# songrise/HyperNeRF-torch

Measured on AMD Instinct MI355X. Metric: ray-samples/sec (fwd+bwd+Adam), whole job; per-GPU = value/n_gpus, higher is better.
Workload: dtype bf16

## Files before the change

hypernerf-torch_amd/csrc/hn_mlp.hip:

```cpp
#include "hn_common.h"
#include <algorithm>
#include <type_traits>

#ifdef HN_PROF
#define HN_STAMP(code)                                                                          \
  do {                                                                                          \
    if (prof_on && prof_n < 2040) {                                                             \
      unsigned long long t__;                                                                   \
      __builtin_amdgcn_sched_barrier(0);                                                        \
      asm volatile("s_memtime %0\n\ts_waitcnt lgkmcnt(0)" : "=s"(t__)::"memory");               \
      __builtin_amdgcn_sched_barrier(0);                                                        \
      if (lane == 0) { prof_buf[2 * prof_n] = (code); prof_buf[2 * prof_n + 1] = (long long)t__; } \
      ++prof_n;                                                                                 \
    }                                                                                           \
  } while (0)
#else
#define HN_STAMP(code) do {} while (0)
#endif

template <int WAVES>
struct WStream {
  const char* g;
  char* lds;
  int ctr;
  int nchunks;
  int wave, lane;

  HN_DEV void issue(int c) {
    const char* src = g + (size_t)c * (HN_CHUNK_UNITS * 1024);
    char* dst = lds + (c & 1) * (HN_CHUNK_UNITS * 1024);
    if constexpr (WAVES == 8) {
      if (wave >= 4) {
        int u0 = wave - 4;
        asm volatile("" : "+s"(u0));
#pragma unroll
        for (int i = 0; i < HN_CHUNK_UNITS / 4; ++i) {
          const int unit = u0 + i * 4;
          __builtin_amdgcn_global_load_lds(
              (const __attribute__((address_space(1))) void*)(src + unit * 1024 + lane * 16),
              (__attribute__((address_space(3))) void*)(dst + unit * 1024), 16, 0, 0);
        }
      }
      return;
    }
#pragma unroll
    for (int i = 0; i < HN_CHUNK_UNITS / WAVES; ++i) {
      const int unit = wave + i * WAVES;
      __builtin_amdgcn_global_load_lds(
          (const __attribute__((address_space(1))) void*)(src + unit * 1024 + lane * 16),
          (__attribute__((address_space(3))) void*)(dst + unit * 1024), 16, 0, 0);
    }
  }
  HN_DEV void start() {
    ctr = 0;
    __syncthreads();
    issue(0);
  }
  HN_DEV const char* take(int n) {
    if ((ctr & (HN_CHUNK_UNITS - 1)) + n > HN_CHUNK_UNITS) ctr = (ctr + HN_CHUNK_UNITS - 1) & ~(HN_CHUNK_UNITS - 1);
    if ((ctr & (HN_CHUNK_UNITS - 1)) == 0) {
      const int c = ctr / HN_CHUNK_UNITS;
      asm volatile("s_waitcnt vmcnt(0)" ::: "memory");
      __syncthreads();
      if (c + 1 < nchunks) issue(c + 1);
    }
    const char* p = lds + (((ctr / HN_CHUNK_UNITS) & 1) * HN_CHUNK_UNITS + (ctr & (HN_CHUNK_UNITS - 1))) * 1024;
    ctr += n;
    return p;
  }
};

#define HN_INV2PI_HI 0.15915494309189535f
#define HN_INV2PI_LO ((float)(0.15915494309189535 - (double)0.15915494309189535f))
// ... 424 lines not shown
    }
    __builtin_amdgcn_sched_barrier(0);
#pragma unroll
    for (int u = 0; u < N; ++u) {
      if (t < NT) {
        acc[t & 1] = hn_mfma_bf16(q[u % D], cur[u], acc[t & 1]);
        if (u + D < N) q[u % D] = *reinterpret_cast<const bf16x8*>(wl + (u + D) * 1024);
      }
      if (t > 0) {
#pragma unroll
        for (int e = 0; e < PER_SLOT; ++e) {
          const int k = u * PER_SLOT + e;
          if (k < SHARES)
            hn_epilogue_share<TRAIN, NT, S8>(k, tp, acc[tp & 1], nxt + tp * 2, bits, out_base, mask_base, lane);
        }
      }
      __builtin_amdgcn_sched_barrier(0);
    }
  }
#pragma unroll
  for (int i = 0; i < NT * 2; ++i) cur[i] = nxt[i];
}

template <bool BF16, int AUXG, bool EXTRA, bool TRAIN, bool S8 = false>
__global__ __launch_bounds__(ModeT<BF16>::WAVES * 64, BF16 ? 2 : 1) void hn_mlp_fwd_kernel(const HnMlpArgs a) {
  using M = ModeT<BF16>;
  constexpr int SX = S8 ? 1 : 0;
  static_assert(!(S8 && (EXTRA || !TRAIN || !BF16)), "the 8-bit stash exists for the render-level bf16 training builds only");
  if constexpr (S8) asm volatile("s_setreg_imm32_b32 hwreg(HW_REG_MODE, 23, 1), 1");
  using Frag = typename M::Frag;
  extern __shared__ __attribute__((aligned(16))) char smem[];
  const int lane = threadIdx.x & 63;
  const int wave = __builtin_amdgcn_readfirstlane(threadIdx.x >> 6);
  const int r = lane & 31, h = lane >> 5;
  constexpr int PTS = M::WAVES * 32;
  const int ntiles = (a.n_points + PTS - 1) / PTS;
  hn_timeline_begin(a.timeline);
#ifdef HN_PROF
  long long* prof_buf = reinterpret_cast<long long*>(a.prof);
  const bool prof_on = prof_buf != nullptr && blockIdx.x == 0 && wave == 0;
  int prof_n = 0;
#endif

  WStream<M::WAVES> ws;
  ws.g = reinterpret_cast<const char*>(a.wstream);
  ws.lds = smem;
  ws.nchunks = a.n_chunks;
  ws.wave = wave;
// ... 17 lines not shown
    feat_lds[i] = e;
    if constexpr (BF16) dfeat_lds[i] = hn_derive_feat_fwd(e, a.n_comps, n_trig, with_lo);
  }
  __syncthreads();

  for (int tile = blockIdx.x; tile < ntiles; tile += gridDim.x) {
    const int blk = tile * M::WAVES + wave;
    const int p0 = blk * 32 + r;
    const bool valid = p0 < a.n_points;
    const int p = valid ? p0 : a.n_points - 1;
    const int ray = p / a.samples_per_ray;
    const bool wave_valid = blk * 32 < a.n_points;
    hn_stage_sources(srcv, a, p, ray, lane, rev, n_trig, with_lo);
    ws.start();

    HnOpWords w_next = hn_load_op(a.ops, 0, a.n_ops);
    for (int op = 0; op < a.n_ops; ++op) {
      const HnOpWords w = w_next;
      w_next = hn_load_op(a.ops, op + 1, a.n_ops);
      const int code = w[0];
      if (code == HN_OP_LAYER) {
        HN_STAMP(100 + op);
        const int K32 = w[1] & 255, nG = (w[1] >> 8) & 255, NT = (w[1] >> 16) & 255;
        const int act = (w[1] >> 24) & 15, flags = (w[1] >> 28) & 15;
        const float* bias = bias_lds + w[2];
        const bool do_mask = TRAIN && w[4] >= 0 && wave_valid && act != HN_ACT_SOFTPLUS;
        const bool do_stash = TRAIN && w[5] >= 0 && wave_valid;
        char* out_base = do_stash ? hn_slot_base<BF16, SX>(a, w[5], NT, blk) : nullptr;
        char* aux_base = (TRAIN && wave_valid) ? hn_slot_base<BF16, SX>(a, w[6], 2 * nG, blk) : nullptr;
        uint32_t* mask_base = do_mask ? hn_mask_base(a, w[4], (NT + 1) >> 1, blk, lane) : nullptr;
        const bool has_out = w_next[0] == HN_OP_OUT;
        const HnOpWords out_w = w_next;
        Frag aux[AUXG * 2 * M::STEPS32];
#pragma unroll
        for (int g = 0; g < AUXG; ++g) {
          if (g < nG) {
            if (EXTRA && (flags & HN_LAYER_DIRECT))
              hn_make_group<true>(aux + g * 2 * M::STEPS32, feat_lds + w[3] + 64 * g, dfeat_lds + w[3] + 64 * g, srcv,
                                  lane, a, p, ray);
            else
              hn_make_group<false>(aux + g * 2 * M::STEPS32, feat_lds + w[3] + 64 * g, dfeat_lds + w[3] + 64 * g, srcv,
                                   lane, a, p, ray);
            if (aux_base != nullptr) {
              hn_stash<BF16, SX>(aux + g * 2 * M::STEPS32, aux_base, 2 * g, lane);
              hn_stash<BF16, SX>(aux + (g * 2 + 1) * M::STEPS32, aux_base, 2 * g + 1, lane);
            }
          }
        }
        unsigned bits = 0;
// ... 3 lines not shown
                             wave_valid && do_stash == do_mask;
          if (plain && K32 == 4 && NT == 4) {
            if (do_stash) hn_layer_pipelined<4, 4, true, SX>(cur, nxt, bias, ws, out_base, mask_base, lane);
            else hn_layer_pipelined<4, 4, false, SX>(cur, nxt, bias, ws, out_base, mask_base, lane);
            continue;
          }
        }
#pragma unroll
        for (int t = 0; t < 8; ++t) {
          if (t < NT) {
            f32x16 acc;
            hn_init_acc(acc, bias, t, h);
            hn_gemm_k<BF16>(acc, cur, K32, ws);
#pragma unroll
            for (int g = 0; g < AUXG; ++g)
              if (g < nG) hn_gemm_blocks<BF16, 2>(acc, aux + g * 2 * M::STEPS32, ws);
            HN_STAMP(2);
            if (act == HN_ACT_RELU) {
#pragma unroll
              for (int i = 0; i < 16; ++i) {
                bits = hn_push_mask<BF16>(bits, acc[i]);
                acc[i] = __int_as_float(max(__float_as_int(acc[i]), 0));
              }
            } else if (act != HN_ACT_NONE) {
              hn_act_tile<BF16>(acc, act, __int_as_float(w[7]), __int_as_float(w[4]), bits);
            }
            if (has_out && t == 0 && h == 0 && valid) {
              const HnDst d = a.dst[out_w[1]];
              const int n = out_w[3];
#pragma unroll
              for (int i = 0; i < 4; ++i) {
                if (i < n) {
                  float y = acc[i];
                  if (out_w[4] == 1) y = 1.0f / (1.0f + expf(-y));
                  if (out_w[5] >= 0) {
                    const HnSrc sr = a.src[out_w[5]];
                    y = __fadd_rn(sr.ptr[(size_t)(sr.per_ray ? ray : p) * sr.ld + out_w[6] + i], y);
                  }
                  d.ptr[(size_t)p * d.ld + out_w[2] + i] = y;
                }
              }
            }
            if (has_out && t == 0 && h == 0 && out_w[7] > 0) {
              const int n = out_w[3];
#pragma unroll
              for (int i = 0; i < 4; ++i) {
                if (i < n) {
// ... 50 lines not shown
            if (t < NT) {
              if constexpr (BF16) {
#pragma unroll
                for (int s = 0; s < 2; ++s)
#pragma unroll
                  for (int j = 0; j < 8; ++j) {
                    const int row = 32 * t + 16 * s + hn_pi16(h, j);
                    if (row < n) d.ptr[(size_t)p * d.ld + w[2] + row] = (float)cur[2 * t + s][j];
                  }
              } else {
#pragma unroll
                for (int q = 0; q < 16; ++q) {
                  const int row = 32 * t + hn_rho(q, h);
                  if (row < n) d.ptr[(size_t)p * d.ld + w[2] + row] = cur[16 * t + q];
                }
              }
            }
        }
      }
    }
  }
  hn_timeline_end(a.timeline);
}

HN_DEV bool hn_prefetch_masks(const HnMlpArgs& a, const HnOpWords& wn, int blk, int lane, bool wave_valid,
                              unsigned* out) {
  if (wn[0] != HN_BOP_LAYER || wn[4] < 0) return false;
  const int NT = (wn[1] >> 16) & 255;
  const uint32_t* mb = hn_mask_base(a, wn[4], (NT + 1) >> 1, blk, lane);
#pragma unroll
  for (int dd = 0; dd < 4; ++dd)
    out[dd] = (2 * dd < NT) ? (wave_valid ? mb[dd * 64 + lane] : 0xffffffffu) : 0u;
  return true;
}

template <bool BF16, bool WIDE, bool S8 = false>
__global__ __launch_bounds__(ModeT<BF16>::WAVES * 64, BF16 ? 2 : 1) void hn_mlp_bwd_kernel(const HnMlpArgs a) {
  using M = ModeT<BF16>;
  constexpr int SZ = S8 ? 2 : 0;
  static_assert(!(S8 && WIDE) && !(S8 && !BF16), "the 8-bit stash exists for the render-level bf16 builds only");
  if constexpr (S8) asm volatile("s_setreg_imm32_b32 hwreg(HW_REG_MODE, 23, 1), 1");
  const float dz_scale = S8 ? ldexpf(1.0f, a.dz_scale_log2) : 1.0f;
  const float dz_unscale = S8 ? ldexpf(1.0f, -a.dz_scale_log2) : 1.0f;
  using Frag = typename M::Frag;
  extern __shared__ __attribute__((aligned(16))) char smem[];
  const int lane = threadIdx.x & 63;
  const int wave = __builtin_amdgcn_readfirstlane(threadIdx.x >> 6);
  const int r = lane & 31, h = lane >> 5;
  constexpr int PTS = M::WAVES * 32;
  const int ntiles = (a.n_points + PTS - 1) / PTS;
  HnFeat* feat_lds = reinterpret_cast<HnFeat*>(smem + 2 * HN_CHUNK_UNITS * 1024);
  HnDFeat* dfeat_lds = reinterpret_cast<HnDFeat*>(feat_lds + ((a.n_feat + 1) & ~1));
  float* srcv = reinterpret_cast<float*>(BF16 ? reinterpret_cast<char*>(dfeat_lds + a.n_feat)
                                              : reinterpret_cast<char*>(dfeat_lds)) + wave * (a.n_comps * 32);
  hn_timeline_begin(a.timeline);
#ifdef HN_PROF
  long long* prof_buf = reinterpret_cast<long long*>(a.prof);
  const bool prof_on = prof_buf != nullptr && blockIdx.x == 0 && wave == 0;
  int prof_n = 0;
#endif
// ... 63 lines not shown
            } else {
              d[i] = 0.0f;
            }
        } else {
#pragma unroll
          for (int i = 0; i < 4; ++i) d[i] = 0.0f;
        }
        Frag tmp[M::STEPS32];
        hn_zero_frags(tmp, M::STEPS32);
        if constexpr (BF16) {
#pragma unroll
          for (int i = 0; i < 4; ++i) tmp[0][i] = (__bf16)d[i];
        } else {
#pragma unroll
          for (int i = 0; i < 4; ++i) tmp[i] = d[i];
        }
        if (a.training && w[7] >= 0 && wave_valid) hn_stash<BF16, SZ>(tmp, hn_slot_base<BF16, SZ>(a, w[7], 1, blk), 0, lane);
#pragma unroll
        for (int s = 0; s < M::STEPS32; ++s) {
          if (to2) cur2[s] = tmp[s];
          else cur[s] = tmp[s];
        }
      } else if (WIDE && code == HN_BOP_LOAD_WIDE) {
        const int n = w[3] & 0xffff, NT = w[4], dact = (w[3] >> 16) & 15;
        const HnSrc s = a.src[w[1]];
        unsigned nbits = 0xffffffffu;
        char* dz_base = (a.training && wave_valid) ? hn_slot_base<BF16>(a, w[7], NT, blk) : nullptr;
        const bool has_mask = w[5] >= 0 && dact != HN_ACT_SOFTPLUS;
        const bool from_y = (dact == HN_ACT_ELU || dact == HN_ACT_SOFTPLUS) && wave_valid;
        const char* y_base = from_y ? hn_slot_base<BF16>(a, w[7], NT, blk) : nullptr;
#pragma unroll
        for (int t = 0; t < 8; ++t) {
          if (t < NT) {
            if (has_mask && !(t & 1)) {
              nbits = wave_valid ? ~hn_mask_base(a, w[5], (NT + 1) >> 1, blk, lane)[(t >> 1) * 64 + lane] : 0u;
            }
            f32x16 v;
            if (dact == 0) {
#pragma unroll
              for (int i = 0; i < 16; ++i) {
                const int row = 32 * t + hn_rho(i, h);
                const bool keep = hn_keep_mask(nbits, t & 1, i) != 0;
                v[i] = (valid && keep && row < n) ? s.ptr[(size_t)p * s.ld + w[2] + row] : 0.0f;
              }
            } else {
              const float p0 = __int_as_float(w[6]), p1 = __int_as_float(w[5]);
              f32x16 y = {0};
              if (y_base != nullptr) y = hn_unstash<BF16>(y_base, t, lane);
#pragma unroll
              for (int i = 0; i < 16; ++i) {
                const int row = 32 * t + hn_rho(i, h);
                const float g = (valid && row < n) ? s.ptr[(size_t)p * s.ld + w[2] + row] : 0.0f;
                float d = 1.0f;
                if (dact == HN_ACT_LEAKY_RELU) d = hn_keep_mask(nbits, t & 1, i) != 0 ? 1.0f : p0;
                else d = hn_dact_y<BF16>(dact, y[i], p0, p1);
                v[i] = g * d;
              }
            }
            hn_acc_to_frags(v, cur + t * M::STEPS32);
            if (dz_base != nullptr) hn_stash<BF16>(cur + t * M::STEPS32, dz_base, t, lane);
          }
        }
      } else if (code == HN_BOP_LAYER) {
        const int K32 = w[1] & 255, K32b = (w[1] >> 8) & 255, NT = (w[1] >> 16) & 255;
        const bool has_mask = w[4] >= 0;
        const bool do_stash = a.training && w[5] >= 0 && wave_valid;
        char* dz_base = do_stash ? hn_slot_base<BF16, SZ>(a, w[5], NT, blk) : nullptr;
        const int dact = w[2];
        const char* y_base = (!S8 && (dact == HN_ACT_ELU || dact == HN_ACT_SOFTPLUS) && wave_valid)
                                 ? hn_slot_base<BF16>(a, w[6], NT, blk) : nullptr;
        unsigned nbits = 0xffffffffu;
        unsigned mbits[4] = {0xffffffffu, 0xffffffffu, 0xffffffffu, 0xffffffffu};
        if (has_mask) {
          if (mnext_ready) {
#pragma unroll
            for (int dd = 0; dd < 4; ++dd) mbits[dd] = ~mnext[dd];
          } else {
            const uint32_t* mb = hn_mask_base(a, w[4], (NT + 1) >> 1, blk, lane);
#pragma unroll
            for (int dd = 0; dd < 4; ++dd)
              if (2 * dd < NT)
                mbits[dd] = wave_valid ? ~mb[dd * 64 + lane] : 0u;
          }
        }
        mnext_ready = false;
#pragma unroll
        for (int t = 0; t < 8; ++t) {
          if (t < NT) {
            f32x16 acc;
            hn_init_acc(acc, nullptr, t, h);
            hn_gemm_k<BF16>(acc, cur, K32, ws);
// ... 71 lines not shown
      for (int i = 0; i < 16; ++i) {
        const int slot = hn_rho(i, h);
        if (slot < a.n_dsrc) a.dsrc[(size_t)p0 * a.n_dsrc + slot] = S8 ? dacc[i] * dz_unscale : dacc[i];
      }
    }
    if (a.embed_reg_mask != 0 && wave_valid) {
      const long long erow = a.embed_idx[(blk * 32) / a.samples_per_ray];
#pragma unroll
      for (int i = 0; i < 16; ++i) {
        if (a.embed_reg_mask & (1 << i)) {
          float v = valid ? (S8 ? dacc[i] * dz_unscale : dacc[i]) : 0.0f;
#pragma unroll
          for (int m = 1; m < 32; m <<= 1) v += __shfl_xor(v, m, 64);
          const int col = a.embed_col[hn_rho(i, h)];
          if (r == 0 && col >= 0) {
            if (!S8 && a.embed_partial != nullptr) a.embed_partial[(size_t)blk * a.embed_dim + col] = v;
            else if (erow >= 0 && erow < a.embed_rows) atomicAdd(a.embed_grad + (size_t)erow * a.embed_dim + col, v);
          }
        }
      }
    }
  }
  hn_timeline_end(a.timeline);
}

#include "hn_pack.h"
template <bool BF16>
__global__ void hn_pack_kernel(const HnPackUnit* units, int n_units, const float* const* ptrs, char* out,
                               const HnPackBias* bias, int n_bias, float* bias_out) {
  hn_pack_one<BF16>(units, n_units, ptrs, out, bias, n_bias, bias_out, blockIdx.x * (blockDim.x >> 6) + (threadIdx.x >> 6));
}
template <bool BF16>
__global__ void hn_pack_multi_kernel(const HnPackTable tab) {
  hn_pack_block<BF16>(tab, (int)blockIdx.x);
}

template <class F>
HN_DEV void static_for4(F&& f) {
  f(std::integral_constant<int, 0>{});
  f(std::integral_constant<int, 1>{});
  f(std::integral_constant<int, 2>{});
  f(std::integral_constant<int, 3>{});
}
template <bool BF16>
struct DwFrag;
typedef __attribute__((ext_vector_type(4))) short s16x4;
// ... 505 lines not shown
  return 8;
}

#define HN_STR2(x) #x
#define HN_STR(x) HN_STR2(x)
extern "C" __attribute__((used)) const char hn_build_config_text[] =
    "HN_BUILD_CONFIG:" HN_STR(HN_WGRAD_STAGES) "," HN_STR(HN_WGRAD_MAXSLOT) ",0," HN_STR(HN_CHUNK_UNITS) ",1,1,"
    HN_STR(HN_BF16_WAVES) "," HN_STR(HN_WGRAD_AUX) ";";
extern "C" int hn_build_config(int32_t* out, int n) {
  const int32_t v[HN_BUILD_CONFIG_N] = {HN_WGRAD_STAGES, HN_WGRAD_MAXSLOT, 0, HN_CHUNK_UNITS,
                                        1,               1,                HN_BF16_WAVES, HN_WGRAD_AUX};
  for (int i = 0; i < n && i < HN_BUILD_CONFIG_N; ++i) out[i] = v[i];
  return HN_BUILD_CONFIG_N;
}

static void hn_allow_big_lds() {
  static bool done[64] = {};
  int dev = 0;
  if (hipGetDevice(&dev) != hipSuccess || dev < 0 || dev >= 64) dev = 0;
  if (done[dev]) return;
  done[dev] = true;
  const int big = 160 * 1024;
#define HN_BIG(k) (void)hipFuncSetAttribute((const void*)(k), hipFuncAttributeMaxDynamicSharedMemorySize, big)
  HN_BIG((hn_mlp_fwd_kernel<true, 2, false, true>)); HN_BIG((hn_mlp_fwd_kernel<true, 2, false, false>));
  HN_BIG((hn_mlp_fwd_kernel<true, 2, true, true>)); HN_BIG((hn_mlp_fwd_kernel<true, 2, true, false>));
  HN_BIG((hn_mlp_fwd_kernel<true, 3, false, true>)); HN_BIG((hn_mlp_fwd_kernel<true, 3, false, false>));
  HN_BIG((hn_mlp_fwd_kernel<true, 3, true, true>)); HN_BIG((hn_mlp_fwd_kernel<true, 3, true, false>));
  HN_BIG((hn_mlp_fwd_kernel<false, 3, true, true>)); HN_BIG((hn_mlp_fwd_kernel<false, 3, true, false>));
  HN_BIG((hn_mlp_fwd_kernel<true, 2, false, true, true>)); HN_BIG((hn_mlp_fwd_kernel<true, 3, false, true, true>));
  HN_BIG((hn_mlp_bwd_kernel<true, false, true>)); HN_BIG((hn_wgrad_kernel<true, true>));
#undef HN_BIG
  (void)hipFuncSetAttribute((const void*)hn_mlp_bwd_kernel<true, false>, hipFuncAttributeMaxDynamicSharedMemorySize, big);
  (void)hipFuncSetAttribute((const void*)hn_mlp_bwd_kernel<true, true>, hipFuncAttributeMaxDynamicSharedMemorySize, big);
  (void)hipFuncSetAttribute((const void*)hn_mlp_bwd_kernel<false, true>, hipFuncAttributeMaxDynamicSharedMemorySize, big);
  (void)hipFuncSetAttribute((const void*)hn_wgrad_kernel<true>, hipFuncAttributeMaxDynamicSharedMemorySize, big);
  (void)hipFuncSetAttribute((const void*)hn_wgrad_kernel<false>, hipFuncAttributeMaxDynamicSharedMemorySize, big);
}

extern "C" int hn_pack_units(int mode, const HnPackUnit* units, int n_units, const float* const* ptrs, void* wstream,
                             const HnPackBias* bias, int n_bias, float* bias_out, hnStream_t stream) {
  if (n_units < 0 || n_bias < 0) return -1;
  const int total = n_units + n_bias;
  if (total == 0) return 0;
  const int grid = (total + 3) / 4;
  if (mode == HN_MODE_BF16 || mode == HN_MODE_BF16_S8)
    hipLaunchKernelGGL(hn_pack_kernel<true>, dim3(grid), dim3(256), 0, (hipStream_t)stream, units, n_units, ptrs,
                       (char*)wstream, bias, n_bias, bias_out);
  else if (mode == HN_MODE_F32)
    hipLaunchKernelGGL(hn_pack_kernel<false>, dim3(grid), dim3(256), 0, (hipStream_t)stream, units, n_units, ptrs,
                       (char*)wstream, bias, n_bias, bias_out);
  else
    return -2;
  HN_CHECK_LAUNCH();
  return 0;
}

extern "C" int hn_pack_units_multi(int mode, const HnPackJob* jobs, int n_jobs, hnStream_t stream) {
  HnPackTable tab = {};
  int blocks = 0;
  const int rc = hn_pack_table_fill(jobs, n_jobs, tab, blocks);
  if (rc != 0) return rc;
  if (blocks == 0) return 0;
  if (mode == HN_MODE_BF16 || mode == HN_MODE_BF16_S8)
    hipLaunchKernelGGL(hn_pack_multi_kernel<true>, dim3(blocks), dim3(256), 0, (hipStream_t)stream, tab);
  else if (mode == HN_MODE_F32)
    hipLaunchKernelGGL(hn_pack_multi_kernel<false>, dim3(blocks), dim3(256), 0, (hipStream_t)stream, tab);
  else
    return -2;
  HN_CHECK_LAUNCH();
  return 0;
}

static int hn_check_args(const HnMlpArgs* a) {
  if (a == nullptr) return -1;
  if (a->n_points <= 0 || a->samples_per_ray <= 0 || a->n_ops <= 0 || a->n_chunks <= 0) return -2;
  if (a->ops == nullptr || a->wstream == nullptr) return -3;
  if (a->mode != HN_MODE_BF16 && a->mode != HN_MODE_F32 && a->mode != HN_MODE_BF16_S8) return -4;
  if (a->mode == HN_MODE_BF16_S8 && a->training && a->wide_ops != 0) return -4;
  if (a->mode == HN_MODE_BF16_S8 && (a->dz_scale_log2 < -60 || a->dz_scale_log2 > 60)) return -5;
  if (a->n_dsrc < 0 || a->n_dsrc > HN_DSRC_COMPS) return -5;
  if (a->n_bias < 0 || a->n_feat < 0 || a->n_comps < 0 || a->n_comps > HN_MAX_COMPS) return -5;
  if (a->max_groups < 0 || a->max_groups > 3) return -5;
  if (a->n_comps > 0 && a->comps == nullptr) return -3;
  return 0;
}

extern "C" int hn_mlp_workspace_bytes(const int32_t* ops_host, int n_ops, int backward, int mode, int64_t n_points,
                                      int64_t* stash_bytes, int64_t* mask_bytes) {
  if (ops_host == nullptr || stash_bytes == nullptr || mask_bytes == nullptr) return -1;
  if (n_ops <= 0 || n_points <= 0) return -2;
  if (mode != HN_MODE_BF16 && mode != HN_MODE_F32 && mode != HN_MODE_BF16_S8) return -4;
  const int64_t nblk = (n_points + 31) / 32;
  const int64_t tile = (mode == HN_MODE_BF16_S8 ? 1 : mode == HN_MODE_BF16 ? ModeT<true>::TILE_UNITS : ModeT<false>::TILE_UNITS) * 1024;
  int64_t sb = 0, mb = 0;
  auto stash = [&](int off_kib, int nt) {
    if (off_kib >= 0) sb = std::max<int64_t>(sb, (int64_t)(unsigned)off_kib * 1024 + nblk * nt * tile);
  };
  auto mask = [&](int off256, int nt_tiles) {
    if (off256 >= 0) mb = std::max<int64_t>(mb, (int64_t)(unsigned)off256 * 256 + nblk * ((nt_tiles + 1) >> 1) * 256);
  };
  for (int i = 0; i < n_ops; ++i) {
    const int32_t* w = ops_host + (size_t)i * HN_OP_WORDS;
    if (!backward) {
      if (w[0] == HN_OP_LAYER) {
        const int nG = (w[1] >> 8) & 255, NT = (w[1] >> 16) & 255, act = (w[1] >> 24) & 15;
        if (act != HN_ACT_SOFTPLUS) mask(w[4], NT);
        stash(w[5], NT);
        stash(w[6], 2 * nG);
      } else if (w[0] != HN_OP_OUT && w[0] != HN_OP_OUT_WIDE) {
        return -7;
      }
    } else {
      if (w[0] == HN_BOP_LOAD) {
        stash(w[7], 1);
      } else if (w[0] == HN_BOP_LOAD_WIDE) {
        if (((w[3] >> 16) & 15) != HN_ACT_SOFTPLUS) mask(w[5], w[4]);
        stash(w[7], w[4]);
      } else if (w[0] == HN_BOP_LAYER) {
        const int NT = (w[1] >> 16) & 255;
        mask(w[4], NT);
        stash(w[5], NT);
        if (w[2] == HN_ACT_ELU || w[2] == HN_ACT_SOFTPLUS) stash(w[6], NT);
      } else if (w[0] != HN_BOP_AUX) {
        return -7;
      }
    }
  }
  *stash_bytes = sb;
  *mask_bytes = mb;
  return 0;
}

extern "C" int hn_mlp_forward(const HnMlpArgs* a, hnStream_t stream) {
  int rc = hn_check_args(a);
  if (rc) return rc;
  hn_allow_big_lds();
  constexpr int WB = ModeT<true>::WAVES;
  if (a->n_trig_comps < 0 || a->n_trig_comps > a->n_comps) return -5;
  const bool bf = a->mode == HN_MODE_BF16 || a->mode == HN_MODE_BF16_S8;
  const size_t planes = bf
                            ? (size_t)a->n_comps + (size_t)a->n_trig_comps + (a->trig_lo_planes ? (size_t)a->n_trig_comps : 1)
                            : (size_t)a->n_comps;
  const size_t lds = 2 * HN_CHUNK_UNITS * 1024 + (size_t)((a->n_bias + 3) & ~3) * 4 +
                     (size_t)((a->n_feat + 1) & ~1) * 8 + (bf ? (size_t)a->n_feat * 16 : 0) +
                     (size_t)8 * planes * 32 * 4;
  if (lds > 158 * 1024) return -6;
  const dim3 grid_b(hn_grid_for(a->n_points, WB * 32)), blk_b(WB * 64);
  const hipStream_t st = (hipStream_t)stream;
#define HN_FWD(G, E, T) hipLaunchKernelGGL((hn_mlp_fwd_kernel<true, G, E, T>), grid_b, blk_b, lds, st, *a)
  if (a->mode == HN_MODE_BF16_S8 && a->training) {
    if (a->max_groups <= 2) hipLaunchKernelGGL((hn_mlp_fwd_kernel<true, 2, false, true, true>), grid_b, blk_b, lds, st, *a);
    else hipLaunchKernelGGL((hn_mlp_fwd_kernel<true, 3, false, true, true>), grid_b, blk_b, lds, st, *a);
  } else if (bf) {
    const bool extra = a->wide_ops != 0, train = a->training != 0;
    if (a->max_groups <= 2) {
      if (extra) { if (train) HN_FWD(2, true, true); else HN_FWD(2, true, false); }
      else { if (train) HN_FWD(2, false, true); else HN_FWD(2, false, false); }
    } else {
      if (extra) { if (train) HN_FWD(3, true, true); else HN_FWD(3, true, false); }
      else { if (train) HN_FWD(3, false, true); else HN_FWD(3, false, false); }
    }
  } else {
    const dim3 grid_f(hn_grid_for(a->n_points, 128)), blk_f(256);
    if (a->training) hipLaunchKernelGGL((hn_mlp_fwd_kernel<false, 3, true, true>), grid_f, blk_f, lds, st, *a);
    else hipLaunchKernelGGL((hn_mlp_fwd_kernel<false, 3, true, false>), grid_f, blk_f, lds, st, *a);
  }
#undef HN_FWD
  HN_CHECK_LAUNCH();
  return 0;
}

extern "C" int hn_mlp_backward(const HnMlpArgs* a, hnStream_t stream) {
  int rc = hn_check_args(a);
  if (rc) return rc;
  hn_allow_big_lds();
  const size_t flds = (size_t)((a->n_feat + 1) & ~1) * 8;
  if (flds > 64 * 1024) return -6;
  if (a->mode == HN_MODE_BF16 || a->mode == HN_MODE_BF16_S8) {
    constexpr int WB = ModeT<true>::WAVES;
    const size_t lds = 2 * HN_CHUNK_UNITS * 1024 + flds + (size_t)a->n_feat * 16 + (size_t)WB * a->n_comps * 32 * 4;
    if (a->mode == HN_MODE_BF16_S8 && a->training)
      hipLaunchKernelGGL((hn_mlp_bwd_kernel<true, false, true>), dim3(hn_grid_for(a->n_points, WB * 32)), dim3(WB * 64), lds,
                         (hipStream_t)stream, *a);
    else if (a->wide_ops & 1)
      hipLaunchKernelGGL((hn_mlp_bwd_kernel<true, true>), dim3(hn_grid_for(a->n_points, WB * 32)), dim3(WB * 64), lds,
                         (hipStream_t)stream, *a);
    else
      hipLaunchKernelGGL((hn_mlp_bwd_kernel<true, false>), dim3(hn_grid_for(a->n_points, WB * 32)), dim3(WB * 64), lds,
                         (hipStream_t)stream, *a);
  } else {
    const size_t lds = 2 * HN_CHUNK_UNITS * 1024 + flds + (size_t)4 * a->n_comps * 32 * 4;
    hipLaunchKernelGGL((hn_mlp_bwd_kernel<false, true>), dim3(hn_grid_for(a->n_points, 128)), dim3(256), lds,
                       (hipStream_t)stream, *a);
  }
  HN_CHECK_LAUNCH();
  return 0;
}

struct HnDwReduceTable {
  float* partials[HN_MAX_WGRAD_BATCH];
  float* grads[HN_MAX_WGRAD_BATCH];
};
struct HnAdamFuseDev {
  float* p; float* g; float* m; float* v;
  const float* hyper; float* step;
  const HnAdamRange* rest;
  int n_rest, zero_grad;
};
#ifndef HN_REDUCE_SPLIT
#define HN_REDUCE_SPLIT 2
#endif
#ifndef HN_REDUCE_INFLIGHT
#define HN_REDUCE_INFLIGHT 8
#endif
template <bool S8, bool ADAM>
// ... 359 lines not shown
```

hypernerf-torch_amd/machine.py:

```python
from __future__ import annotations

import os
import weakref

import ctypes as C
import itertools
import math
from dataclasses import dataclass, field
from typing import Dict, List, Optional, Sequence, Tuple

import numpy as np
import torch

from . import _lib as L

CHUNK = L.HN_CHUNK_UNITS


def pow2ceil(n: int) -> int:
    p = 1
    while p < n:
        p *= 2
    return p


def bf16_like(mode: int) -> bool:
    return mode in (L.HN_MODE_BF16, L.HN_MODE_BF16_S8)


def mode_consts(mode: int):
    if mode == L.HN_MODE_BF16_S8:
        return 2, 1024
    return (2, 2048) if mode == L.HN_MODE_BF16 else (4, 4096)


DZ_SCALE_LOG2 = int(os.environ.get("HN_DZ_SCALE_LOG2", 16))


ACT_CODES = {"none": L.HN_ACT_NONE, "relu": L.HN_ACT_RELU, "leaky_relu": L.HN_ACT_LEAKY_RELU, "elu": L.HN_ACT_ELU,
             "softplus": L.HN_ACT_SOFTPLUS}
MASK_ACTS = ("relu", "leaky_relu")
Y_ACTS = ("elu", "softplus")


def f32_bits(x: float) -> int:
    return int(np.array([x], dtype=np.float32).view(np.int32)[0])


@dataclass
class Feature:
    src: int
    comp: int
    kind: int
    freq: float = 1.0
    need_grad: bool = False


def posenc_features(src: int, comps: Sequence[int], n_freqs: int, need_grad: bool = False) -> List[Feature]:
    out = [Feature(src, c, L.HN_FEAT_ID, 1.0, need_grad) for c in comps]
# ... 303 lines not shown
                        p1 if ly.act == "softplus" else ly.mask_slot, ly.out_slot, aux_slot, p0])
            if ly.out is not None:
                o = ly.out
                if o.wide:
                    if not ly.commit:
                        raise ValueError("wide outputs are read from the committed activation")
                    ops.append([L.HN_OP_OUT_WIDE, o.dst, o.col, ly.n_out, ly.nt, 0, 0, 0])
                else:
                    ops.append([L.HN_OP_OUT, o.dst, o.col, ly.n_out, 1 if o.act == "sigmoid" else 0,
                                o.residual[0] if o.residual else -1, o.residual[1] if o.residual else 0,
                                o.publish_ci + 1 if o.publish is not None else 0])
        return np.asarray(ops, dtype=np.int32)

    @staticmethod
    def _dact(ly: Layer) -> Tuple[int, int, int]:
        if ly.act in ("none", "relu"):
            return 0, 0, 0
        return ACT_CODES[ly.act], f32_bits(ly.act_params[0]), f32_bits(ly.act_params[1])

    @property
    def y_acts(self) -> bool:
        return any(ly.act in Y_ACTS for ly in self.layers)

    def _aux_grad_groups(self, ly: Layer) -> List[int]:
        if ly.aux is None:
            return []
        return [g for g in range(ly.aux.groups) if any(f.need_grad for f in ly.aux.feats[64 * g:64 * g + 64])]

    @staticmethod
    def _aux_tile_word(ly: Layer, g: int) -> int:
        word = 0
        for tt in range(2):
            fts = [f for f in ly.aux.feats[64 * g + 32 * tt:64 * g + 32 * tt + 32] if f.need_grad]
            if fts:
                word |= 1 << tt
            if any(f.kind not in (L.HN_FEAT_ID, L.HN_FEAT_ZERO) for f in fts):
                word |= 256 << tt
        return word

    def _build_bwd_ops(self) -> np.ndarray:
        ops, plan = [], []

        def emit_load(ly: Layer, to2: bool):
            gi = ly.grad_in
            if gi is None:
                raise ValueError(f"{ly.name}: output layer without a gradient source")
# ... 760 lines not shown
    def pack(self, device, mode, force: bool = False):
        d = self._tables(device, mode)
        need, key = self._needs_pack(d, force)
        if not need:
            return d
        d.pack_backward = BACKWARD_SERIAL[0]
        self._pack_job(d, device)
        L.launch("hn_pack_units", C.c_int(mode), L.ptr(d.units), C.c_int(d.n_units), L.ptr(d.ptrs), L.ptr(d.wstream),
                 L.ptr(d.bias_desc), C.c_int(d.n_bias), L.ptr(d.bias), L.stream_handle(), tag=self.prog.name)
        d.pack_key = key
        return d

    def _args(self, d, mode, n_points, samples_per_ray, training, ops, n_ops, wstream_ptr, n_chunks, srcs, dsts,
              stash, masks, dsrc, embed=None, kind="hn_mlp_forward"):
        a = L.HnMlpArgs()
        a.mode, a.n_points, a.samples_per_ray, a.training = mode, n_points, samples_per_ray, int(training)
        a.n_ops, a.n_chunks, a.n_dsrc = n_ops, n_chunks, self.prog.n_dsrc if dsrc is not None else 0
        a.ops, a.wstream, a.bias, a.feat = ops.data_ptr(), wstream_ptr, d.bias.data_ptr(), d.feat.data_ptr()
        a.n_bias, a.n_feat = max(32, self.prog.bias_len), max(1, len(self.prog.feat_table))
        a.max_groups = max([ly.aux.groups for ly in self.prog.layers if ly.aux is not None], default=0)
        a.prof = L.PROF_BUFFER.data_ptr() if L.PROF_BUFFER is not None else 0
        a.timeline = L.timeline_slot(f"{kind}[{self.prog.name}]", d.bias.device)
        a.comps, a.n_comps = d.comps.data_ptr(), len(self.prog.comp_map)
        wide = any(ly.out is not None and ly.out.wide for ly in self.prog.layers)
        direct = any(f.kind != L.HN_FEAT_ZERO and (f.src, f.comp) not in self.prog.comp_map for f in self.prog.feat_table)
        a.wide_ops = (1 if wide else 0) | (2 if direct else 0)
        a.dz_scale_log2 = DZ_SCALE_LOG2 if mode == L.HN_MODE_BF16_S8 else 0
        a.n_trig_comps = min(len(self.prog.comp_map), max(1, self.prog.n_trig_comps))
        n_feat, n_bias = max(1, len(self.prog.feat_table)), max(32, self.prog.bias_len)
        fixed = 2 * CHUNK * 1024 + ((n_bias + 3) & ~3) * 4 + ((n_feat + 1) & ~1) * 8 + n_feat * 16
        full = fixed + 8 * (a.n_comps + 2 * a.n_trig_comps) * 128
        a.trig_lo_planes = 1 if full <= 158 * 1024 else 0
        a.stash = stash.data_ptr() if stash is not None else 0
        a.masks = masks.data_ptr() if masks is not None else 0
        a.dsrc = dsrc.data_ptr() if dsrc is not None else 0
        for i, s in enumerate(srcs):
            if s is None:
                continue
            t, per_ray = s[0], s[1]
            L.require_gpu(t)
            if t.dtype != torch.float32 or t.stride(-1) != 1:
                raise L.HnError("sources must be fp32 with unit inner stride")
            a.src[i].ptr, a.src[i].ld, a.src[i].per_ray = t.data_ptr(), t.stride(-2) if t.dim() > 1 else 1, int(per_ray)
            if len(s) > 2 and s[2] is not None:
                idx = s[2]
                L.require_gpu(idx)
                if idx.dtype != torch.int64 or not idx.is_contiguous():
                    raise L.HnError("gather indices must be contiguous int64")
                a.src[i].gather_idx, a.src[i].gather_rows = idx.data_ptr(), t.shape[0]
        if embed is not None:
            g_tab, idx, src_i = embed[:3]
            if len(embed) > 3 and embed[3] is not None:
                a.embed_partial = embed[3].data_ptr()
            mask, col = self.prog.embed_fold(src_i)
            a.embed_reg_mask, a.embed_grad, a.embed_idx = mask, g_tab.data_ptr(), idx.data_ptr()
            a.embed_rows, a.embed_dim = g_tab.shape[0], g_tab.shape[1]
            for k in range(L.HN_DSRC_COMPS):
                a.embed_col[k] = col[k]
        for i, t in enumerate(dsts):
            if t is None:
                continue
            L.require_gpu(t)
            a.dst[i].ptr, a.dst[i].ld = t.data_ptr(), t.stride(-2) if t.dim() > 1 else 1
        return a

    def _ops(self, device, mode, n_points):
        key = ("ops", str(device), mode, n_points)
        hit = self._jobs.get(key)
        if hit is None:
            fwd, bwd = self.prog.resolved_ops(mode, n_points)
            hit = (L.to_device_bytes(fwd, device), L.to_device_bytes(bwd, device))
            self._jobs[key] = hit
        return hit

    @staticmethod
    def _job_bytes(mode: int) -> int:
        return WGRAD_JOB_BYTES // 2 if mode == L.HN_MODE_BF16_S8 else WGRAD_JOB_BYTES

    def effective_mode(self, mode: int) -> int:
        if mode == L.HN_MODE_BF16_S8:
            wide = any(ly.out is not None and ly.out.wide for ly in self.prog.layers)
            direct = any(f.kind != L.HN_FEAT_ZERO and (f.src, f.comp) not in self.prog.comp_map
                         for f in self.prog.feat_table)
            if wide or direct:
                return L.HN_MODE_BF16
        return mode

    def forward(self, mode, n_points, samples_per_ray, srcs, dsts, training: bool):
        mode = self.effective_mode(mode)
        if mode == L.HN_MODE_BF16_S8 and training and self.prog.y_acts:
            raise NotImplementedError(
                f"{self.prog.name}: precision 'bf16s8' keeps the training stash in 8 bits, too coarse to take the "
                "derivative of an ELU / Softplus layer from its output; use 'bf16' or 'fp32' (LeakyReLU works: it needs "
# ... 74 lines not shown
```

Baseline: 80.94 million.

## Specialize MLP kernels for relu-only nets and read args from kernarg segment

```diff
diff --git a/hypernerf-torch_amd/csrc/hn_mlp.hip b/hypernerf-torch_amd/csrc/hn_mlp.hip
--- a/hypernerf-torch_amd/csrc/hn_mlp.hip
+++ b/hypernerf-torch_amd/csrc/hn_mlp.hip
@@ -26,29 +26,19 @@
   int nchunks;
   int wave, lane;
 
+  static constexpr int ISSUERS = WAVES == 8 ? 4 : WAVES;
   HN_DEV void issue(int c) {
-    const char* src = g + (size_t)c * (HN_CHUNK_UNITS * 1024);
-    char* dst = lds + (c & 1) * (HN_CHUNK_UNITS * 1024);
-    if constexpr (WAVES == 8) {
-      if (wave >= 4) {
-        int u0 = wave - 4;
-        asm volatile("" : "+s"(u0));
-#pragma unroll
-        for (int i = 0; i < HN_CHUNK_UNITS / 4; ++i) {
-          const int unit = u0 + i * 4;
-          __builtin_amdgcn_global_load_lds(
-              (const __attribute__((address_space(1))) void*)(src + unit * 1024 + lane * 16),
-              (__attribute__((address_space(3))) void*)(dst + unit * 1024), 16, 0, 0);
-        }
-      }
-      return;
-    }
-#pragma unroll
-    for (int i = 0; i < HN_CHUNK_UNITS / WAVES; ++i) {
-      const int unit = wave + i * WAVES;
-      __builtin_amdgcn_global_load_lds(
-          (const __attribute__((address_space(1))) void*)(src + unit * 1024 + lane * 16),
-          (__attribute__((address_space(3))) void*)(dst + unit * 1024), 16, 0, 0);
+    if (WAVES == 8 && wave < 4) return;
+    const int u0 = WAVES == 8 ? wave - 4 : wave;
+    const char* src = g + ((size_t)c * HN_CHUNK_UNITS + u0) * 1024;
+    char* dst = lds + ((c & 1) * HN_CHUNK_UNITS + u0) * 1024;
+    const unsigned voff = lane * 16;
+#pragma unroll 1
+    for (int i = 0; i < HN_CHUNK_UNITS / ISSUERS; ++i) {
+      __builtin_amdgcn_global_load_lds((const __attribute__((address_space(1))) void*)(src + voff),
+                                       (__attribute__((address_space(3))) void*)dst, 16, 0, 0);
+      src += ISSUERS * 1024;
+      dst += ISSUERS * 1024;
     }
   }
   HN_DEV void start() {
@@ -519,8 +509,8 @@
   for (int i = 0; i < NT * 2; ++i) cur[i] = nxt[i];
 }
 
-template <bool BF16, int AUXG, bool EXTRA, bool TRAIN, bool S8 = false>
-__global__ __launch_bounds__(ModeT<BF16>::WAVES * 64, BF16 ? 2 : 1) void hn_mlp_fwd_kernel(const HnMlpArgs a) {
+template <bool BF16, int AUXG, bool EXTRA, bool TRAIN, bool S8, bool ACTS>
+HN_DEV void hn_mlp_fwd_body(const HnMlpArgs& a) {
   using M = ModeT<BF16>;
   constexpr int SX = S8 ? 1 : 0;
   static_assert(!(S8 && (EXTRA || !TRAIN || !BF16)), "the 8-bit stash exists for the render-level bf16 training builds only");
@@ -584,9 +574,9 @@
       if (code == HN_OP_LAYER) {
         HN_STAMP(100 + op);
         const int K32 = w[1] & 255, nG = (w[1] >> 8) & 255, NT = (w[1] >> 16) & 255;
-        const int act = (w[1] >> 24) & 15, flags = (w[1] >> 28) & 15;
+        const int act = ACTS ? (w[1] >> 24) & 15 : (w[1] >> 24) & 1, flags = (w[1] >> 28) & 15;
         const float* bias = bias_lds + w[2];
-        const bool do_mask = TRAIN && w[4] >= 0 && wave_valid && act != HN_ACT_SOFTPLUS;
+        const bool do_mask = TRAIN && w[4] >= 0 && wave_valid && (!ACTS || act != HN_ACT_SOFTPLUS);
         const bool do_stash = TRAIN && w[5] >= 0 && wave_valid;
         char* out_base = do_stash ? hn_slot_base<BF16, SX>(a, w[5], NT, blk) : nullptr;
         char* aux_base = (TRAIN && wave_valid) ? hn_slot_base<BF16, SX>(a, w[6], 2 * nG, blk) : nullptr;
@@ -636,7 +626,7 @@
                 bits = hn_push_mask<BF16>(bits, acc[i]);
                 acc[i] = __int_as_float(max(__float_as_int(acc[i]), 0));
               }
-            } else if (act != HN_ACT_NONE) {
+            } else if (ACTS && act != HN_ACT_NONE) {
               hn_act_tile<BF16>(acc, act, __int_as_float(w[7]), __int_as_float(w[4]), bits);
             }
             if (has_out && t == 0 && h == 0 && valid) {
@@ -733,6 +723,17 @@
   }
   hn_timeline_end(a.timeline);
 }
+HN_DEV const HnMlpArgs& hn_kernel_args() {
+  return *(const HnMlpArgs*)(const __attribute__((address_space(4))) HnMlpArgs*)__builtin_amdgcn_kernarg_segment_ptr();
+}
+template <bool BF16, int AUXG, bool EXTRA, bool TRAIN, bool S8 = false>
+__global__ __launch_bounds__(ModeT<BF16>::WAVES * 64, BF16 ? 2 : 1) void hn_mlp_fwd_kernel(const HnMlpArgs) {
+  hn_mlp_fwd_body<BF16, AUXG, EXTRA, TRAIN, S8, false>(hn_kernel_args());
+}
+template <bool BF16, int AUXG, bool EXTRA, bool TRAIN, bool S8 = false>
+__global__ __launch_bounds__(ModeT<BF16>::WAVES * 64, BF16 ? 2 : 1) void hn_mlp_fwd_act_kernel(const HnMlpArgs) {
+  hn_mlp_fwd_body<BF16, AUXG, EXTRA, TRAIN, S8, true>(hn_kernel_args());
+}
 
 HN_DEV bool hn_prefetch_masks(const HnMlpArgs& a, const HnOpWords& wn, int blk, int lane, bool wave_valid,
                               unsigned* out) {
@@ -745,8 +746,8 @@
   return true;
 }
 
-template <bool BF16, bool WIDE, bool S8 = false>
-__global__ __launch_bounds__(ModeT<BF16>::WAVES * 64, BF16 ? 2 : 1) void hn_mlp_bwd_kernel(const HnMlpArgs a) {
+template <bool BF16, bool WIDE, bool S8, bool ACTS>
+HN_DEV void hn_mlp_bwd_body(const HnMlpArgs& a) {
   using M = ModeT<BF16>;
   constexpr int SZ = S8 ? 2 : 0;
   static_assert(!(S8 && WIDE) && !(S8 && !BF16), "the 8-bit stash exists for the render-level bf16 builds only");
@@ -856,7 +857,7 @@
           else cur[s] = tmp[s];
         }
       } else if (WIDE && code == HN_BOP_LOAD_WIDE) {
-        const int n = w[3] & 0xffff, NT = w[4], dact = (w[3] >> 16) & 15;
+        const int n = w[3] & 0xffff, NT = w[4], dact = ACTS ? (w[3] >> 16) & 15 : 0;
         const HnSrc s = a.src[w[1]];
         unsigned nbits = 0xffffffffu;
         char* dz_base = (a.training && wave_valid) ? hn_slot_base<BF16>(a, w[7], NT, blk) : nullptr;
@@ -900,7 +901,7 @@
         const bool has_mask = w[4] >= 0;
         const bool do_stash = a.training && w[5] >= 0 && wave_valid;
         char* dz_base = do_stash ? hn_slot_base<BF16, SZ>(a, w[5], NT, blk) : nullptr;
-        const int dact = w[2];
+        const int dact = ACTS ? w[2] : 0;
         const char* y_base = (!S8 && (dact == HN_ACT_ELU || dact == HN_ACT_SOFTPLUS) && wave_valid)
                                  ? hn_slot_base<BF16>(a, w[6], NT, blk) : nullptr;
         unsigned nbits = 0xffffffffu;
@@ -1018,6 +1019,14 @@
     }
   }
   hn_timeline_end(a.timeline);
+}
+template <bool BF16, bool WIDE, bool S8 = false>
+__global__ __launch_bounds__(ModeT<BF16>::WAVES * 64, BF16 ? 2 : 1) void hn_mlp_bwd_kernel(const HnMlpArgs) {
+  hn_mlp_bwd_body<BF16, WIDE, S8, false>(hn_kernel_args());
+}
+template <bool BF16, bool WIDE, bool S8 = false>
+__global__ __launch_bounds__(ModeT<BF16>::WAVES * 64, BF16 ? 2 : 1) void hn_mlp_bwd_act_kernel(const HnMlpArgs) {
+  hn_mlp_bwd_body<BF16, WIDE, S8, true>(hn_kernel_args());
 }
 
 #include "hn_pack.h"
@@ -1569,19 +1578,18 @@
   done[dev] = true;
   const int big = 160 * 1024;
 #define HN_BIG(k) (void)hipFuncSetAttribute((const void*)(k), hipFuncAttributeMaxDynamicSharedMemorySize, big)
-  HN_BIG((hn_mlp_fwd_kernel<true, 2, false, true>)); HN_BIG((hn_mlp_fwd_kernel<true, 2, false, false>));
-  HN_BIG((hn_mlp_fwd_kernel<true, 2, true, true>)); HN_BIG((hn_mlp_fwd_kernel<true, 2, true, false>));
-  HN_BIG((hn_mlp_fwd_kernel<true, 3, false, true>)); HN_BIG((hn_mlp_fwd_kernel<true, 3, false, false>));
-  HN_BIG((hn_mlp_fwd_kernel<true, 3, true, true>)); HN_BIG((hn_mlp_fwd_kernel<true, 3, true, false>));
-  HN_BIG((hn_mlp_fwd_kernel<false, 3, true, true>)); HN_BIG((hn_mlp_fwd_kernel<false, 3, true, false>));
-  HN_BIG((hn_mlp_fwd_kernel<true, 2, false, true, true>)); HN_BIG((hn_mlp_fwd_kernel<true, 3, false, true, true>));
-  HN_BIG((hn_mlp_bwd_kernel<true, false, true>)); HN_BIG((hn_wgrad_kernel<true, true>));
+#define HN_BIG2(k, ...) HN_BIG((k##_kernel<__VA_ARGS__>)); HN_BIG((k##_act_kernel<__VA_ARGS__>))
+  HN_BIG2(hn_mlp_fwd, true, 2, false, true); HN_BIG2(hn_mlp_fwd, true, 2, false, false);
+  HN_BIG2(hn_mlp_fwd, true, 2, true, true); HN_BIG2(hn_mlp_fwd, true, 2, true, false);
+  HN_BIG2(hn_mlp_fwd, true, 3, false, true); HN_BIG2(hn_mlp_fwd, true, 3, false, false);
+  HN_BIG2(hn_mlp_fwd, true, 3, true, true); HN_BIG2(hn_mlp_fwd, true, 3, true, false);
+  HN_BIG((hn_mlp_fwd_act_kernel<false, 3, true, true>)); HN_BIG((hn_mlp_fwd_act_kernel<false, 3, true, false>));
+  HN_BIG2(hn_mlp_fwd, true, 2, false, true, true); HN_BIG2(hn_mlp_fwd, true, 3, false, true, true);
+  HN_BIG2(hn_mlp_bwd, true, false, true); HN_BIG2(hn_mlp_bwd, true, false); HN_BIG2(hn_mlp_bwd, true, true);
+  HN_BIG((hn_mlp_bwd_act_kernel<false, true>));
+  HN_BIG((hn_wgrad_kernel<true, true>)); HN_BIG((hn_wgrad_kernel<true>)); HN_BIG((hn_wgrad_kernel<false>));
+#undef HN_BIG2
 #undef HN_BIG
-  (void)hipFuncSetAttribute((const void*)hn_mlp_bwd_kernel<true, false>, hipFuncAttributeMaxDynamicSharedMemorySize, big);
-  (void)hipFuncSetAttribute((const void*)hn_mlp_bwd_kernel<true, true>, hipFuncAttributeMaxDynamicSharedMemorySize, big);
-  (void)hipFuncSetAttribute((const void*)hn_mlp_bwd_kernel<false, true>, hipFuncAttributeMaxDynamicSharedMemorySize, big);
-  (void)hipFuncSetAttribute((const void*)hn_wgrad_kernel<true>, hipFuncAttributeMaxDynamicSharedMemorySize, big);
-  (void)hipFuncSetAttribute((const void*)hn_wgrad_kernel<false>, hipFuncAttributeMaxDynamicSharedMemorySize, big);
 }
 
 extern "C" int hn_pack_units(int mode, const HnPackUnit* units, int n_units, const float* const* ptrs, void* wstream,
@@ -1623,7 +1631,7 @@
   if (a->n_points <= 0 || a->samples_per_ray <= 0 || a->n_ops <= 0 || a->n_chunks <= 0) return -2;
   if (a->ops == nullptr || a->wstream == nullptr) return -3;
   if (a->mode != HN_MODE_BF16 && a->mode != HN_MODE_F32 && a->mode != HN_MODE_BF16_S8) return -4;
-  if (a->mode == HN_MODE_BF16_S8 && a->training && a->wide_ops != 0) return -4;
+  if (a->mode == HN_MODE_BF16_S8 && a->training && (a->wide_ops & 3) != 0) return -4;
   if (a->mode == HN_MODE_BF16_S8 && (a->dz_scale_log2 < -60 || a->dz_scale_log2 > 60)) return -5;
   if (a->n_dsrc < 0 || a->n_dsrc > HN_DSRC_COMPS) return -5;
   if (a->n_bias < 0 || a->n_feat < 0 || a->n_comps < 0 || a->n_comps > HN_MAX_COMPS) return -5;
@@ -1636,7 +1644,10 @@
                                       int64_t* stash_bytes, int64_t* mask_bytes) {
   if (ops_host == nullptr || stash_bytes == nullptr || mask_bytes == nullptr) return -1;
   if (n_ops <= 0 || n_points <= 0) return -2;
+  const bool acts_stated = ((mode >> 8) & 4) != 0;
+  mode &= 255;
   if (mode != HN_MODE_BF16 && mode != HN_MODE_F32 && mode != HN_MODE_BF16_S8) return -4;
+  auto check_act = [&](int act) { return act == HN_ACT_NONE || act == HN_ACT_RELU || acts_stated; };
   const int64_t nblk = (n_points + 31) / 32;
   const int64_t tile = (mode == HN_MODE_BF16_S8 ? 1 : mode == HN_MODE_BF16 ? ModeT<true>::TILE_UNITS : ModeT<false>::TILE_UNITS) * 1024;
   int64_t sb = 0, mb = 0;
@@ -1651,6 +1662,7 @@
     if (!backward) {
       if (w[0] == HN_OP_LAYER) {
         const int nG = (w[1] >> 8) & 255, NT = (w[1] >> 16) & 255, act = (w[1] >> 24) & 15;
+        if (!check_act(act)) return -9;
         if (act != HN_ACT_SOFTPLUS) mask(w[4], NT);
         stash(w[5], NT);
         stash(w[6], 2 * nG);
@@ -1661,10 +1673,12 @@
       if (w[0] == HN_BOP_LOAD) {
         stash(w[7], 1);
       } else if (w[0] == HN_BOP_LOAD_WIDE) {
+        if (!check_act((w[3] >> 16) & 15)) return -9;
         if (((w[3] >> 16) & 15) != HN_ACT_SOFTPLUS) mask(w[5], w[4]);
         stash(w[7], w[4]);
       } else if (w[0] == HN_BOP_LAYER) {
         const int NT = (w[1] >> 16) & 255;
+        if (!check_act(w[2])) return -9;
         mask(w[4], NT);
         stash(w[5], NT);
         if (w[2] == HN_ACT_ELU || w[2] == HN_ACT_SOFTPLUS) stash(w[6], NT);
@@ -1694,12 +1708,17 @@
   if (lds > 158 * 1024) return -6;
   const dim3 grid_b(hn_grid_for(a->n_points, WB * 32)), blk_b(WB * 64);
   const hipStream_t st = (hipStream_t)stream;
-#define HN_FWD(G, E, T) hipLaunchKernelGGL((hn_mlp_fwd_kernel<true, G, E, T>), grid_b, blk_b, lds, st, *a)
+  const bool acts = (a->wide_ops & 4) != 0;
+#define HN_FWD(...)                                                                                              \
+  do {                                                                                                           \
+    if (acts) hipLaunchKernelGGL((hn_mlp_fwd_act_kernel<true, __VA_ARGS__>), grid_b, blk_b, lds, st, *a);        \
+    else hipLaunchKernelGGL((hn_mlp_fwd_kernel<true, __VA_ARGS__>), grid_b, blk_b, lds, st, *a);                 \
+  } while (0)
   if (a->mode == HN_MODE_BF16_S8 && a->training) {
-    if (a->max_groups <= 2) hipLaunchKernelGGL((hn_mlp_fwd_kernel<true, 2, false, true, true>), grid_b, blk_b, lds, st, *a);
-    else hipLaunchKernelGGL((hn_mlp_fwd_kernel<true, 3, false, true, true>), grid_b, blk_b, lds, st, *a);
+    if (a->max_groups <= 2) HN_FWD(2, false, true, true);
+    else HN_FWD(3, false, true, true);
   } else if (bf) {
-    const bool extra = a->wide_ops != 0, train = a->training != 0;
+    const bool extra = (a->wide_ops & 3) != 0, train = a->training != 0;
     if (a->max_groups <= 2) {
       if (extra) { if (train) HN_FWD(2, true, true); else HN_FWD(2, true, false); }
       else { if (train) HN_FWD(2, false, true); else HN_FWD(2, false, false); }
@@ -1709,8 +1728,8 @@
     }
   } else {
     const dim3 grid_f(hn_grid_for(a->n_points, 128)), blk_f(256);
-    if (a->training) hipLaunchKernelGGL((hn_mlp_fwd_kernel<false, 3, true, true>), grid_f, blk_f, lds, st, *a);
-    else hipLaunchKernelGGL((hn_mlp_fwd_kernel<false, 3, true, false>), grid_f, blk_f, lds, st, *a);
+    if (a->training) hipLaunchKernelGGL((hn_mlp_fwd_act_kernel<false, 3, true, true>), grid_f, blk_f, lds, st, *a);
+    else hipLaunchKernelGGL((hn_mlp_fwd_act_kernel<false, 3, true, false>), grid_f, blk_f, lds, st, *a);
   }
 #undef HN_FWD
   HN_CHECK_LAUNCH();
@@ -1726,18 +1745,21 @@
   if (a->mode == HN_MODE_BF16 || a->mode == HN_MODE_BF16_S8) {
     constexpr int WB = ModeT<true>::WAVES;
     const size_t lds = 2 * HN_CHUNK_UNITS * 1024 + flds + (size_t)a->n_feat * 16 + (size_t)WB * a->n_comps * 32 * 4;
-    if (a->mode == HN_MODE_BF16_S8 && a->training)
-      hipLaunchKernelGGL((hn_mlp_bwd_kernel<true, false, true>), dim3(hn_grid_for(a->n_points, WB * 32)), dim3(WB * 64), lds,
-                         (hipStream_t)stream, *a);
-    else if (a->wide_ops & 1)
-      hipLaunchKernelGGL((hn_mlp_bwd_kernel<true, true>), dim3(hn_grid_for(a->n_points, WB * 32)), dim3(WB * 64), lds,
-                         (hipStream_t)stream, *a);
-    else
-      hipLaunchKernelGGL((hn_mlp_bwd_kernel<true, false>), dim3(hn_grid_for(a->n_points, WB * 32)), dim3(WB * 64), lds,
-                         (hipStream_t)stream, *a);
+    const dim3 grid_b(hn_grid_for(a->n_points, WB * 32)), blk_b(WB * 64);
+    const hipStream_t st = (hipStream_t)stream;
+    const bool acts = (a->wide_ops & 4) != 0;
+#define HN_BWD(...)                                                                                              \
+  do {                                                                                                           \
+    if (acts) hipLaunchKernelGGL((hn_mlp_bwd_act_kernel<true, __VA_ARGS__>), grid_b, blk_b, lds, st, *a);        \
+    else hipLaunchKernelGGL((hn_mlp_bwd_kernel<true, __VA_ARGS__>), grid_b, blk_b, lds, st, *a);                 \
+  } while (0)
+    if (a->mode == HN_MODE_BF16_S8 && a->training) HN_BWD(false, true);
+    else if (a->wide_ops & 1) HN_BWD(true);
+    else HN_BWD(false);
+#undef HN_BWD
   } else {
     const size_t lds = 2 * HN_CHUNK_UNITS * 1024 + flds + (size_t)4 * a->n_comps * 32 * 4;
-    hipLaunchKernelGGL((hn_mlp_bwd_kernel<false, true>), dim3(hn_grid_for(a->n_points, 128)), dim3(256), lds,
+    hipLaunchKernelGGL((hn_mlp_bwd_act_kernel<false, true>), dim3(hn_grid_for(a->n_points, 128)), dim3(256), lds,
                        (hipStream_t)stream, *a);
   }
   HN_CHECK_LAUNCH();
diff --git a/hypernerf-torch_amd/machine.py b/hypernerf-torch_amd/machine.py
--- a/hypernerf-torch_amd/machine.py
+++ b/hypernerf-torch_amd/machine.py
@@ -35,6 +35,7 @@
 
 
 DZ_SCALE_LOG2 = int(os.environ.get("HN_DZ_SCALE_LOG2", 16))
+FORCE_ACT_BUILD = os.environ.get("HN_FORCE_ACT_BUILD") == "1"
 
 
 ACT_CODES = {"none": L.HN_ACT_NONE, "relu": L.HN_ACT_RELU, "leaky_relu": L.HN_ACT_LEAKY_RELU, "elu": L.HN_ACT_ELU,
@@ -384,6 +385,10 @@
     def y_acts(self) -> bool:
         return any(ly.act in Y_ACTS for ly in self.layers)
 
+    @property
+    def beyond_relu(self) -> bool:
+        return any(ly.act not in ("none", "relu") for ly in self.layers)
+
     def _aux_grad_groups(self, ly: Layer) -> List[int]:
         if ly.aux is None:
             return []
@@ -1190,9 +1195,7 @@
         a.prof = L.PROF_BUFFER.data_ptr() if L.PROF_BUFFER is not None else 0
         a.timeline = L.timeline_slot(f"{kind}[{self.prog.name}]", d.bias.device)
         a.comps, a.n_comps = d.comps.data_ptr(), len(self.prog.comp_map)
-        wide = any(ly.out is not None and ly.out.wide for ly in self.prog.layers)
-        direct = any(f.kind != L.HN_FEAT_ZERO and (f.src, f.comp) not in self.prog.comp_map for f in self.prog.feat_table)
-        a.wide_ops = (1 if wide else 0) | (2 if direct else 0)
+        a.wide_ops = self.wide_ops()
         a.dz_scale_log2 = DZ_SCALE_LOG2 if mode == L.HN_MODE_BF16_S8 else 0
         a.n_trig_comps = min(len(self.prog.comp_map), max(1, self.prog.n_trig_comps))
         n_feat, n_bias = max(1, len(self.prog.feat_table)), max(32, self.prog.bias_len)
@@ -1232,11 +1235,25 @@
             a.dst[i].ptr, a.dst[i].ld = t.data_ptr(), t.stride(-2) if t.dim() > 1 else 1
         return a
 
+    def wide_ops(self) -> int:
+        wide = any(ly.out is not None and ly.out.wide for ly in self.prog.layers)
+        direct = any(f.kind != L.HN_FEAT_ZERO and (f.src, f.comp) not in self.prog.comp_map for f in self.prog.feat_table)
+        acts = self.prog.beyond_relu or FORCE_ACT_BUILD
+        return (1 if wide else 0) | (2 if direct else 0) | (4 if acts else 0)
+
     def _ops(self, device, mode, n_points):
         key = ("ops", str(device), mode, n_points)
         hit = self._jobs.get(key)
         if hit is None:
             fwd, bwd = self.prog.resolved_ops(mode, n_points)
+            for back, ops in ((0, fwd), (1, bwd)):
+                ops_h = np.ascontiguousarray(ops, dtype=np.int32)
+                sb, mb = C.c_int64(), C.c_int64()
+                rc = L.load().hn_mlp_workspace_bytes(ops_h.ctypes.data_as(C.c_void_p), C.c_int(len(ops_h)), C.c_int(back),
+                                                     C.c_int(mode | self.wide_ops() << 8), C.c_int64(n_points),
+                                                     C.byref(sb), C.byref(mb))
+                if rc != 0:
+                    raise L.HnError(f"{self.prog.name}: hn_mlp_workspace_bytes refuses the op program (rc {rc})")
             hit = (L.to_device_bytes(fwd, device), L.to_device_bytes(bwd, device))
             self._jobs[key] = hit
         return hit
```

Result: no change. 80.77 million (-0.2%).
